# mrluin/TextualDegRemoval

Hardware: AMD Instinct MI355X
Metric: train images/sec (512x512, bs=4/GPU) (higher is better)
Workload: dtype f32 (3xbf16-split MFMA: 24-bit operand significands on the full fp32 exponent range, fp32 accumulate; unscaled gradients, no loss scale, no step-skip guard; tensors fp32 -- the MASA-encoder ResidualBlock activations / gradients as three bf16 planes whose sum IS the fp32 value, bit for bit)

## Files before the change

### textualdegremoval_amd/csrc/tdr_common.h

```cpp
#pragma once
#include <hip/hip_runtime.h>
#include <stdint.h>
#include <stdio.h>
#include <string.h>

#define TDR_OK 0
#define TDR_ERR_ARG (-1)
#define TDR_ERR_HIP (-2)
#define TDR_ERR_UNSUPPORTED (-3)

void tdr_set_error(const char* fmt, ...);

#define TDR_REQUIRE(cond, ...)                     \
    do {                                           \
        if (!(cond)) {                             \
            tdr_set_error(__VA_ARGS__);            \
            return TDR_ERR_ARG;                    \
        }                                          \
    } while (0)

#define TDR_LAUNCH_CHECK(name)                                                         \
    do {                                                                               \
        hipError_t e__ = hipGetLastError();                                            \
        if (e__ != hipSuccess) {                                                       \
            tdr_set_error("%s: launch failed: %s", name, hipGetErrorString(e__));      \
            return TDR_ERR_HIP;                                                        \
        }                                                                              \
    } while (0)

struct TdrConvDesc;
int tdr_conv_forward_bx3(const TdrConvDesc* d, void* stream);

static inline int tdr_cdiv(long a, long b) { return (int)((a + b - 1) / b); }

#include <stdlib.h>
#ifdef TDR_TUNING_KNOBS
static inline const char* tdr_tune_env(const char* name) { return getenv(name); }
#else
static inline const char* tdr_tune_env(const char*) { return nullptr; }
#endif

typedef __attribute__((ext_vector_type(16))) float f32x16;
typedef __attribute__((ext_vector_type(4))) float f32x4;

__device__ __forceinline__ float wave_sum(float v) {
#pragma unroll
    for (int o = 32; o > 0; o >>= 1) v += __shfl_xor(v, o, 64);
    return v;
}
template <int CTRL>
__device__ __forceinline__ float dpp_perm(float v) {
    return __builtin_bit_cast(float, __builtin_amdgcn_update_dpp(0, __builtin_bit_cast(int, v), CTRL, 0xf, 0xf, true));
}
__device__ __forceinline__ float wave_sum_dpp(float v) {
    v += dpp_perm<0xB1>(v);
    v += dpp_perm<0x4E>(v);
    v += dpp_perm<0x141>(v);
    v += dpp_perm<0x140>(v);
    const int b = __builtin_bit_cast(int, v);
    return (__builtin_bit_cast(float, __builtin_amdgcn_readlane(b, 0)) + __builtin_bit_cast(float, __builtin_amdgcn_readlane(b, 16))) +
           (__builtin_bit_cast(float, __builtin_amdgcn_readlane(b, 32)) + __builtin_bit_cast(float, __builtin_amdgcn_readlane(b, 48)));
}
__device__ __forceinline__ float wave_max(float v) {
#pragma unroll
    for (int o = 32; o > 0; o >>= 1) v = fmaxf(v, __shfl_xor(v, o, 64));
    return v;
}

typedef float tdr_f32x2 __attribute__((ext_vector_type(2)));
typedef _Float16 tdr_f16x2 __attribute__((ext_vector_type(2)));
template <bool PIN = true>
__device__ __forceinline__ void tdr_split2_f16(float x0, float x1, unsigned& h, unsigned& m) {
    if constexpr (PIN) asm volatile("" : "+v"(x0), "+v"(x1));
    const tdr_f32x2 xv = {x0, x1};
    h = __builtin_bit_cast(unsigned, __builtin_convertvector(xv, tdr_f16x2));
    const float neg1 = -1.0f;
    asm("v_fma_mixlo_f16 %0, %1, %2, %3 op_sel:[0,0,0] op_sel_hi:[1,0,0]" : "=v"(m) : "v"(h), "v"(neg1), "v"(x0));
    asm("v_fma_mixhi_f16 %0, %1, %2, %3 op_sel:[1,0,0] op_sel_hi:[1,0,0]" : "+v"(m) : "v"(h), "v"(neg1), "v"(x1));
}

typedef __bf16 tdr_bf16x2 __attribute__((ext_vector_type(2)));
template <bool PIN = true>
__device__ __forceinline__ void tdr_split3_bf16(float x0, float x1, unsigned& h, unsigned& m, unsigned& l) {
    if constexpr (PIN) asm volatile("" : "+v"(x0), "+v"(x1));
    const tdr_f32x2 xv = {x0, x1};
    h = __builtin_bit_cast(unsigned, __builtin_convertvector(xv, tdr_bf16x2));
    const float r0 = x0 - __builtin_bit_cast(float, h << 16), r1 = x1 - __builtin_bit_cast(float, h & 0xffff0000u);
    const tdr_f32x2 rv = {r0, r1};
    m = __builtin_bit_cast(unsigned, __builtin_convertvector(rv, tdr_bf16x2));
    const tdr_f32x2 sv = {r0 - __builtin_bit_cast(float, m << 16), r1 - __builtin_bit_cast(float, m & 0xffff0000u)};
    l = __builtin_bit_cast(unsigned, __builtin_convertvector(sv, tdr_bf16x2));
}
```

### textualdegremoval_amd/csrc/tdr_conv_mfma.hip

```cpp
#include "tdr_common.h"
#include "tdr_conv_epi.h"
#include "tdr_pack.h"
#include "../../include/tdr.h"

namespace {

constexpr int cmax(int a, int b) { return a > b ? a : b; }
constexpr int plane_elems(int NT, int TW, int KH, int S, int D) {
    return (((NT * 32 / TW) - 1) * S + (KH - 1) * D + 1) * ((TW - 1) * S + (KH - 1) * D + 1);
}
constexpr int max_plane(int NT, int KH, int S, int D) {
    return cmax(plane_elems(NT, 8, KH, S, D), cmax(plane_elems(NT, 16, KH, S, D), plane_elems(NT, 32, KH, S, D)));
}

template <int KH, int S, int D, int CK, int WM, int TM, int TN, int EPI, bool GATE>
__global__ __launch_bounds__(256) void conv_mfma_kernel(ConvArgs a) {
    constexpr int WN = 4 / WM;
    constexpr int BM = 32 * TM * WM;
    constexpr int NT = TN * WN;
    constexpr int TAPS = KH * KH;
    constexpr int KC = CK * TAPS;
    constexpr int MAXPIT = (max_plane(NT, KH, S, D) + 63) / 64;
    constexpr int CPW = CK / 4;
    constexpr int W4 = KC * BM / 4;
// ... 96 lines not shown
    const int abase = kk * BM + wm * TM * 32 + j;

    f32x16 acc[TM][TN];
#pragma unroll
    for (int tm = 0; tm < TM; ++tm)
#pragma unroll
        for (int tn = 0; tn < TN; ++tn)
#pragma unroll
            for (int r = 0; r < 16; ++r) acc[tm][tn][r] = 0.f;

    load_chunk(0);
    for (int ch = 0; ch < nchunks; ++ch) {
        {
            __syncthreads();
            store_chunk(ch);
            __syncthreads();
        }
        if (ch + 1 < nchunks) load_chunk(ch + 1);
#pragma unroll
        for (int tap = 0; tap < TAPS; ++tap) {
            const int tapoff = (tap / KH) * D * LW + (tap % KH) * D;
#pragma unroll
            for (int c2 = 0; c2 < CK / 2; ++c2) {
                float af[TM], bf[TN];
#pragma unroll
                for (int tm = 0; tm < TM; ++tm)
                    af[tm] = s_w[abase + (tap * CK + 2 * c2) * BM + tm * 32];
#pragma unroll
                for (int tn = 0; tn < TN; ++tn)
                    bf[tn] = s_in[bbase[tn] + 2 * c2 * plane + tapoff];
#pragma unroll
                for (int tm = 0; tm < TM; ++tm)
#pragma unroll
                    for (int tn = 0; tn < TN; ++tn)
                        acc[tm][tn] = __builtin_amdgcn_mfma_f32_32x32x2f32(af[tm], bf[tn], acc[tm][tn], 0, 0, 0);
            }
        }
    }

    conv_epilogue<TM, TN, EPI>(a, acc, n, m0, wm, wn, oy0, ox0, j, kk);
}

template <int KH, int S, int D, int CK, int WM, int TM, int TN, int EPI, bool GATE>
int launch_cfg(const ConvArgs& a, int N, hipStream_t st) {
    constexpr int WN = 4 / WM;
    constexpr int BM = 32 * TM * WM;
    constexpr int NT = TN * WN;
    constexpr int KC = CK * KH * KH;
    const int TW = 1 << a.tw_log2, SR = 32 >> a.tw_log2, TH = NT * SR;
    const int LH = (TH - 1) * S + (KH - 1) * D + 1, LW = (TW - 1) * S + (KH - 1) * D + 1;
    const size_t lds = (size_t)(KC * BM + CK * LH * LW) * sizeof(float);
    ConvArgs b = a;
    b.tiles_x = tdr_cdiv(a.OW, TW);
    const int tiles_y = tdr_cdiv(a.OH, TH);
    dim3 grid(b.tiles_x * tiles_y, tdr_cdiv(a.Cout, BM), N);
    auto kern = conv_mfma_kernel<KH, S, D, CK, WM, TM, TN, EPI, GATE>;
    static bool attr_set = false;
    if (!attr_set) {
        (void)hipFuncSetAttribute(reinterpret_cast<const void*>(kern), hipFuncAttributeMaxDynamicSharedMemorySize, 160 * 1024);
        attr_set = true;
    }
    hipLaunchKernelGGL(kern, grid, dim3(256), lds, st, b);
    TDR_LAUNCH_CHECK("conv_mfma_kernel");
    return TDR_OK;
}

template <int KH, int S, int D, int CK, int EPI, bool GATE>
int launch_shape(const ConvArgs& a, int N, hipStream_t st) {
    const long pix = (long)a.OH * a.OW;
    auto blocks = [&](int bm, int bn) { return (long)tdr_cdiv(a.Cout, bm) * tdr_cdiv(pix, bn) * N; };
    if (a.Cout <= 32) {
        if (blocks(32, 256) < 256) return launch_cfg<KH, S, D, CK, 1, 1, 1, EPI, GATE>(a, N, st);
        return launch_cfg<KH, S, D, CK, 1, 1, 2, EPI, GATE>(a, N, st);
    }
    if (a.Cout > 64 && blocks(128, 128) >= 512) return launch_cfg<KH, S, D, CK, 2, 2, 2, EPI, GATE>(a, N, st);
    if (blocks(64, 128) >= 512) return launch_cfg<KH, S, D, CK, 2, 1, 2, EPI, GATE>(a, N, st);
    return launch_cfg<KH, S, D, CK, 2, 1, 1, EPI, GATE>(a, N, st);
}

__global__ void pack_weights_kernel(const float* __restrict__ w, int Cout, int Cin, int KH, int mode, int CK,
                                    int M, int Kch, int KHe, int Mpad, long total, float* __restrict__ wp) {
    for (long i = blockIdx.x * (long)blockDim.x + threadIdx.x; i < total; i += (long)gridDim.x * blockDim.x)
        wp[i] = tdr_pack_f32_elem(w, Cin, KH, mode, CK, M, Kch, KHe, Mpad, i);
}

__global__ void pack_patches_kernel(const float* __restrict__ blk, int G, int C, int BH, int BW, int PH, int PW, int pstep,
                                    int dil, int off, int CK, int Mpad, long per_b, long total, float* __restrict__ wp) {
    for (long i = blockIdx.x * (long)blockDim.x + threadIdx.x; i < total; i += (long)gridDim.x * blockDim.x) {
        const long b = i / per_b;
        long r = i % per_b;
        const int m = (int)(r % Mpad); r /= Mpad;
        const int ck = (int)(r % CK); r /= CK;
        const int tap = (int)(r % 9);
        const int chunk = (int)(r / 9);
        const int c = chunk * CK + ck;
        float v = 0.f;
        if (m < G * PH * PW && c < C) {
            const int g = m / (PH * PW), q = m % (PH * PW);
            const int py = q / PW, px = q % PW;
            const int y = py * pstep + (tap / 3) * dil + off, x = px * pstep + (tap % 3) * dil + off;
            v = blk[(((b * G + g) * C + c) * BH + y) * BW + x];
        }
        wp[i] = v;
    }
}

}

extern "C" int tdr_conv_ck(int KH_eff) { return KH_eff == 1 ? 32 : (KH_eff == 2 ? 16 : 8); }

extern "C" int64_t tdr_packed_weight_floats(int M, int Kch, int KH_eff) {
    const int CK = tdr_conv_ck(KH_eff);
    const long Mpad = (M + 31) / 32 * 32;
    return (long)((Kch + CK - 1) / CK) * KH_eff * KH_eff * CK * Mpad;
}

extern "C" int tdr_pack_weights(const float* w, int Cout, int Cin, int KH, int mode, float* wp, void* stream) {
    TDR_REQUIRE(w && wp, "tdr_pack_weights: null pointer");
    TDR_REQUIRE(mode >= 0 && mode <= 3, "tdr_pack_weights: bad mode %d", mode);
    int M, Kch, KHe;
    if (mode == 0) { M = Cout; Kch = Cin; KHe = KH; }
    else if (mode == 1) { M = Cin; Kch = Cout; KHe = KH; }
    else if (mode == 2) { TDR_REQUIRE(KH == 2, "mode 2 needs a 2x2 kernel"); M = 4 * Cin; Kch = Cout; KHe = 1; }
    else { TDR_REQUIRE(KH == 3, "mode 3 needs a 3x3 kernel"); M = 4 * Cin; Kch = Cout; KHe = 2; }
    const int CK = tdr_conv_ck(KHe);
    const int Mpad = (M + 31) / 32 * 32;
    const long total = tdr_packed_weight_floats(M, Kch, KHe);
    const int blocks = (int)((total + 255) / 256 < 4096 ? (total + 255) / 256 : 4096);
    hipLaunchKernelGGL(pack_weights_kernel, dim3(blocks), dim3(256), 0, (hipStream_t)stream, w, Cout, Cin, KH, mode, CK,
                       M, Kch, KHe, Mpad, total, wp);
    TDR_LAUNCH_CHECK("pack_weights_kernel");
    return TDR_OK;
}

extern "C" int tdr_pack_patches(const float* blk, int B, int G, int C, int BH, int BW, int PH, int PW, int pstep, int dil,
                                int off, float* wp, void* stream) {
    TDR_REQUIRE(blk && wp, "tdr_pack_patches: null pointer");
    const int CK = 8;
    const int Mpad = (G * PH * PW + 31) / 32 * 32;
    const long per_b = (long)((C + CK - 1) / CK) * 9 * CK * Mpad;
    const long total = per_b * B;
    const int blocks = (int)((total + 255) / 256 < 8192 ? (total + 255) / 256 : 8192);
    hipLaunchKernelGGL(pack_patches_kernel, dim3(blocks), dim3(256), 0, (hipStream_t)stream, blk, G, C, BH, BW, PH, PW,
                       pstep, dil, off, CK, Mpad, per_b, total, wp);
    TDR_LAUNCH_CHECK("pack_patches_kernel");
    return TDR_OK;
}

extern "C" int tdr_conv_forward(const TdrConvDesc* d, void* stream) {
    TDR_REQUIRE(d && d->in && d->wp && d->out, "tdr_conv_forward: null pointer");
    TDR_REQUIRE(d->N > 0 && d->Cin > 0 && d->Cout > 0 && d->OH > 0 && d->OW > 0, "tdr_conv_forward: bad shape");
    TDR_REQUIRE(d->Mpad % 32 == 0 && d->Mpad >= d->Cout, "tdr_conv_forward: Mpad %d invalid for Cout %d", d->Mpad, d->Cout);
    TDR_REQUIRE(d->epi != EPI_GATEBWD || d->aux, "tdr_conv_forward: GATEBWD needs aux");
    if (d->wp_fmt >= 1 && d->wp_fmt <= 3) return tdr_conv_forward_bx3(d, stream);
    TDR_REQUIRE(d->wp_fmt == 0, "tdr_conv_forward: unknown wp_fmt %d", d->wp_fmt);
    ConvArgs a;
    a.in = d->in; a.in_ns = d->in_ns; a.Cin = d->Cin; a.H = d->H; a.W = d->W;
    a.wp = (const float*)d->wp; a.wp_ns = d->wp_ns; a.Mpad = d->Mpad; a.Cout = d->Cout;
    a.out = d->out; a.out_ns = d->out_ns; a.OH = d->OH; a.OW = d->OW;
    a.pad = d->pad;
    a.tw_log2 = d->OW >= 24 ? 5 : (d->OW >= 12 ? 4 : 3);
    a.tiles_x = 0;
    a.kscale = d->kscale; a.kscale_ns = d->kscale_ns;
    a.gate_off = (long)d->Cin * d->H * d->W;
    a.bias = d->bias; a.bias_ns = d->bias_ns; a.scale = d->scale; a.scale_ns = d->scale_ns;
    a.bias2 = d->bias2; a.bias2_ns = d->bias2_ns; a.bias2_mul = d->bias2_mul;
    a.res = d->res; a.res_ns = d->res_ns; a.mask = d->mask; a.mask_ns = d->mask_ns;
    a.aux = d->aux; a.aux_ns = d->aux_ns; a.relu = d->relu;
    a.vec_epi = 0; a.single_buf = 0; a.scheme = 0;
    hipStream_t st = (hipStream_t)stream;
    const int N = d->N;
    const int key = d->KH * 1000 + d->stride * 100 + d->dil * 10 + d->epi;
    const bool g = d->gate != 0;
    switch (key) {
        case 1110: return g ? launch_shape<1, 1, 1, 32, EPI_STD, true>(a, N, st)
                            : launch_shape<1, 1, 1, 32, EPI_STD, false>(a, N, st);
        case 1111: if (!g) return launch_shape<1, 1, 1, 32, EPI_GATEBWD, false>(a, N, st); break;
        case 1112: if (!g) return launch_shape<1, 1, 1, 32, EPI_PSHUF, false>(a, N, st); break;
        case 3110: if (!g) return launch_shape<3, 1, 1, 8, EPI_STD, false>(a, N, st); break;
        case 3112: if (!g) return launch_shape<3, 1, 1, 8, EPI_PSHUF, false>(a, N, st); break;
        case 3120: if (!g) return launch_shape<3, 1, 2, 8, EPI_STD, false>(a, N, st); break;
        case 3130: if (!g) return launch_shape<3, 1, 3, 8, EPI_STD, false>(a, N, st); break;
        case 3210: if (!g) return launch_shape<3, 2, 1, 8, EPI_STD, false>(a, N, st); break;
        case 2210: if (!g) return launch_shape<2, 2, 1, 16, EPI_STD, false>(a, N, st); break;
        case 2112: if (!g) return launch_shape<2, 1, 1, 16, EPI_PSHUF, false>(a, N, st); break;
        default: break;
    }
    tdr_set_error("tdr_conv_forward: unsupported (KH=%d stride=%d dil=%d epi=%d gate=%d)", d->KH, d->stride, d->dil,
                  d->epi, d->gate);
    return TDR_ERR_UNSUPPORTED;
}

namespace {
__global__ __launch_bounds__(256) void pack_multi_kernel(const TdrPackJob* __restrict__ jobs, int n_jobs) {
    int lo = 0, hi = n_jobs - 1;
    while (lo < hi) {
        const int mid = (lo + hi + 1) >> 1;
        if (jobs[mid].first_block <= (long)blockIdx.x) lo = mid; else hi = mid - 1;
    }
    const TdrPackJob jb = jobs[lo];
    const long i = ((long)blockIdx.x - jb.first_block) * 256 + threadIdx.x;
    if (i >= jb.total) return;
    if (jb.fmt == 0)
        reinterpret_cast<float*>(jb.wp)[i] = tdr_pack_f32_elem(jb.w, jb.Cin, jb.KH, jb.mode, jb.CK, jb.M, jb.Kch, jb.KHe, jb.Mx, i);
    else if (jb.fmt == 1 && jb.KHe == 3 && jb.mode == 0)
        tdr_pack_bx3_alltaps9<0>(jb.w, jb.Cin, jb.M, jb.Kch, jb.Mx, i, reinterpret_cast<uint4*>(jb.wp));
    else if (jb.fmt == 1 && jb.KHe == 3 && jb.mode == 1)
        tdr_pack_bx3_alltaps9<1>(jb.w, jb.Cin, jb.M, jb.Kch, jb.Mx, i, reinterpret_cast<uint4*>(jb.wp));
    else if (jb.fmt == 1)
        tdr_pack_bx3_frag(jb.w, jb.Cin, jb.KH, jb.mode, jb.M, jb.Kch, jb.KHe, jb.Mx, i, reinterpret_cast<uint4*>(jb.wp));
    else if (jb.mode == 0 && jb.KHe == 1)
        tdr_pack_hx2_fwd_alltaps<1>(jb.w, jb.Cin, jb.M, jb.Kch, jb.Mx, i, reinterpret_cast<uint4*>(jb.wp));
    else if (jb.mode == 0 && jb.KHe == 2)
        tdr_pack_hx2_fwd_alltaps<4>(jb.w, jb.Cin, jb.M, jb.Kch, jb.Mx, i, reinterpret_cast<uint4*>(jb.wp));
    else if (jb.mode == 0 && jb.KHe == 3)
        tdr_pack_hx2_fwd_alltaps<9>(jb.w, jb.Cin, jb.M, jb.Kch, jb.Mx, i, reinterpret_cast<uint4*>(jb.wp));
    else
        tdr_pack_hx2_frag(jb.w, jb.Cin, jb.KH, jb.mode, jb.M, jb.Kch, jb.KHe, jb.Mx, i, reinterpret_cast<uint4*>(jb.wp));
}
}

extern "C" int tdr_pack_job_init(TdrPackJob* job, const float* w, int Cout, int Cin, int KH, int mode, int fmt, void* wp) {
    TDR_REQUIRE(job && w && wp, "tdr_pack_job_init: null pointer");
    TDR_REQUIRE(mode >= 0 && mode <= 3 && fmt >= 0 && fmt <= 2, "tdr_pack_job_init: bad mode/fmt");
    int M, Kch, KHe;
    if (mode == 0) { M = Cout; Kch = Cin; KHe = KH; }
    else if (mode == 1) { M = Cin; Kch = Cout; KHe = KH; }
    else if (mode == 2) { TDR_REQUIRE(KH == 2, "mode 2 needs a 2x2 kernel"); M = 4 * Cin; Kch = Cout; KHe = 1; }
    else { TDR_REQUIRE(KH == 3, "mode 3 needs a 3x3 kernel"); M = 4 * Cin; Kch = Cout; KHe = 2; }
    job->w = w; job->wp = wp; job->Cout = Cout; job->Cin = Cin; job->KH = KH; job->mode = mode; job->fmt = fmt;
    job->M = M; job->Kch = Kch; job->KHe = KHe;
    if (fmt == 0) {
        job->CK = tdr_conv_ck(KHe);
        job->Mx = (M + 31) / 32 * 32;
        job->total = tdr_packed_weight_floats(M, Kch, KHe);
    } else {
        job->CK = 16;
        job->Mx = (M + 31) / 32;
        job->total = (long)((Kch + 15) / 16) * KHe * KHe * job->Mx * 64;
        if (fmt == 2 && mode == 0 && KHe >= 1 && KHe <= 3) job->total = (long)((Kch + 15) / 16) * job->Mx * 64;
        if (fmt == 1 && KHe == 3 && mode <= 1) job->total = (long)((Kch + 15) / 16) * job->Mx * 64;
    }
    job->first_block = 0;
    return TDR_OK;
}

extern "C" int tdr_pack_weights_multi(const TdrPackJob* jobs_dev, int n_jobs, int64_t total_blocks, void* stream) {
    TDR_REQUIRE(jobs_dev && n_jobs > 0 && total_blocks > 0 && total_blocks < (1LL << 31), "tdr_pack_weights_multi: bad argument");
    hipLaunchKernelGGL(pack_multi_kernel, dim3((unsigned)total_blocks), dim3(256), 0, (hipStream_t)stream, jobs_dev, n_jobs);
    TDR_LAUNCH_CHECK("pack_multi_kernel");
    return TDR_OK;
}
```

### textualdegremoval_amd/csrc/tdr_wgrad_common.h

```cpp
#pragma once
#include "tdr_common.h"

struct TdrWgradDesc;

struct WgArgs {
    const float* in; long in_ns; int Cin, H, W; long gate_off;
    const float* dout; long dout_ns; int Cout, OH, OW;
    int pad, tw_log2, tiles_x, tiles_y, tpi , tps , spi ;
    float* part;
    float* dbpart;
    int scheme;
    const void* grp_tab;
    int grp_bpp;
    int grp_pairs;
};

struct WgPlan { int tw_log2, tiles_x, tiles_y, tpi, tps, spi, cfg, WKw, BMc, BNc; };

bool tdr_wgrad_bx3_supported(const TdrWgradDesc* d);
WgPlan tdr_wgrad_bx3_plan(const TdrWgradDesc* d);
int tdr_wgrad_bx3_launch(const WgArgs& a, const WgPlan& p, const TdrWgradDesc* d, hipStream_t st);

bool tdr_wgrad_s2_supported(const TdrWgradDesc* d);
WgPlan tdr_wgrad_s2_plan(const TdrWgradDesc* d);
int tdr_wgrad_s2_launch(const WgArgs& a, const WgPlan& p, const TdrWgradDesc* d, hipStream_t st);

bool tdr_wgrad_1x1_supported(const TdrWgradDesc* d);
WgPlan tdr_wgrad_1x1_plan(const TdrWgradDesc* d);
int tdr_wgrad_1x1_launch(const WgArgs& a, const WgPlan& p, const TdrWgradDesc* d, hipStream_t st);
```

### textualdegremoval_amd/csrc/tdr_wgrad_mfma.hip

```cpp
#include <stdio.h>
#include <stdlib.h>
#include "tdr_common.h"
#include "tdr_wgrad_common.h"
#include "../../include/tdr.h"

namespace {

constexpr int wg_plane(int TW, int KH, int S) { return (((64 / TW) - 1) * S + KH) * ((TW - 1) * S + KH); }
constexpr int wg_cmax(int a, int b) { return a > b ? a : b; }
constexpr int wg_max_plane(int KH, int S) {
    return wg_cmax(wg_plane(8, KH, S), wg_cmax(wg_plane(16, KH, S), wg_plane(32, KH, S)));
}

template <int KH, int S, int WMw, int WNw, int WKw, int TMW, int TNW, bool GATE>
__global__ __launch_bounds__(256) void wgrad_mfma_kernel(WgArgs a) {
    static_assert(WMw * WNw * WKw == 4, "4 waves");
    constexpr int TAPS = KH * KH;
    constexpr int BMc = 32 * TMW * WMw, BNc = 32 * TNW * WNw;
    constexpr int MAXPIT = (wg_max_plane(KH, S) + 63) / 64;
    constexpr int DPT = BMc / 4;
    constexpr int IPT = BNc / 4;
    constexpr int KPW = 32 / WKw;

    extern __shared__ __attribute__((aligned(16))) float smem[];
// ... 30 lines not shown
    for (int i = 0; i < DPT; ++i) rdsum[i] = 0.f;
    float ri[IPT][MAXPIT];
    float ri2[GATE ? IPT : 1][GATE ? MAXPIT : 1];
    bool dok_r = false;
    unsigned iok_r = 0;
    auto load_tile = [&](int t) {
        const int ty = t / a.tiles_x, tx = t % a.tiles_x;
        const int oy0 = ty * (64 >> a.tw_log2), ox0 = tx * TW;
        const int oy = oy0 + dpy, ox = ox0 + dpx;
        dok_r = oy < a.OH && ox < a.OW;
        const long doff = dok_r ? (long)oy * a.OW + ox : 0;
#pragma unroll
        for (int i = 0; i < DPT; ++i) {
            const int co = min(co0 + wave + 4 * i, a.Cout - 1);
            rd[i] = do_n[(long)co * HWo + doff];
        }
        const int iy0 = oy0 * S - a.pad, ix0 = ox0 * S - a.pad;
        iok_r = 0;
#pragma unroll
        for (int it = 0; it < MAXPIT; ++it) {
            const int gy = iy0 + pr[it], gx = ix0 + pc[it];
            const bool ok = pr[it] >= 0 && gy >= 0 && gy < a.H && gx >= 0 && gx < a.W;
            iok_r |= (ok ? 1u : 0u) << it;
            const long off = ok ? (long)gy * a.W + gx : 0;
#pragma unroll
            for (int i = 0; i < IPT; ++i) {
                const int ci = min(ci0 + wave + 4 * i, a.Cin - 1);
                ri[i][it] = in_n[(long)ci * HWin + off];
                if (GATE) ri2[i][it] = in_n[(long)ci * HWin + off + a.gate_off];
            }
        }
    };
    auto store_tile = [&]() {
#pragma unroll
        for (int i = 0; i < DPT; ++i) {
            const float dv = (dok_r && co0 + wave + 4 * i < a.Cout) ? rd[i] : 0.f;
            s_d[(wave + 4 * i) * 65 + lane] = dv;
            rdsum[i] += dv;
        }
#pragma unroll
        for (int it = 0; it < MAXPIT; ++it)
            if (pr[it] >= 0) {
#pragma unroll
                for (int i = 0; i < IPT; ++i) {
                    float v = ri[i][it];
                    if (GATE) v *= ri2[i][it];
                    s_i[(wave + 4 * i) * planeP + lane + 64 * it] =
                        (((iok_r >> it) & 1u) && ci0 + wave + 4 * i < a.Cin) ? v : 0.f;
                }
            }
    };

    f32x16 acc[TMW][TNW][TAPS];
#pragma unroll
    for (int x = 0; x < TMW; ++x)
#pragma unroll
        for (int y = 0; y < TNW; ++y)
#pragma unroll
            for (int t = 0; t < TAPS; ++t)
#pragma unroll
                for (int r = 0; r < 16; ++r) acc[x][y][t][r] = 0.f;

    const int abase = (wm * TMW * 32 + j) * 65 + kk;
    const int bbase = (wn * TNW * 32 + j) * planeP + kk * S;

    if (t_begin < t_end) load_tile(t_begin);
    for (int t = t_begin; t < t_end; ++t) {
        __syncthreads();
        store_tile();
        __syncthreads();
        if (t + 1 < t_end) load_tile(t + 1);
#pragma unroll
        for (int q = 0; q < KPW; ++q) {
            const int k2 = wk * KPW + q;
            const int p0 = 2 * k2;
            const int py0 = p0 >> a.tw_log2, px0 = p0 & (TW - 1);
            const int pixoff = py0 * S * LW + px0 * S;
            float af[TMW];
#pragma unroll
            for (int x = 0; x < TMW; ++x) af[x] = s_d[abase + x * 32 * 65 + p0];
#pragma unroll
            for (int tap = 0; tap < TAPS; ++tap) {
                const int toff = pixoff + (tap / KH) * LW + (tap % KH);
#pragma unroll
                for (int y = 0; y < TNW; ++y) {
                    const float bf = s_i[bbase + y * 32 * planeP + toff];
#pragma unroll
                    for (int x = 0; x < TMW; ++x)
                        acc[x][y][tap] = __builtin_amdgcn_mfma_f32_32x32x2f32(af[x], bf, acc[x][y][tap], 0, 0, 0);
                }
            }
        }
    }

    if (a.dbpart && blockIdx.z == 0) {
#pragma unroll
        for (int i = 0; i < DPT; ++i) {
            const float sv = wave_sum(rdsum[i]);
            const int co = co0 + wave + 4 * i;
            if (lane == 0 && co < a.Cout) a.dbpart[(long)split * a.Cout + co] = sv;
        }
    }
    float* part = a.part + ((long)split * WKw + wk) * a.Cout * a.Cin * TAPS;
#pragma unroll
    for (int x = 0; x < TMW; ++x)
#pragma unroll
        for (int y = 0; y < TNW; ++y) {
            const int ci = ci0 + (wn * TNW + y) * 32 + j;
            if (ci >= a.Cin) continue;
#pragma unroll
            for (int r = 0; r < 16; ++r) {
                const int co = co0 + (wm * TMW + x) * 32 + (r & 3) + 8 * (r >> 2) + 4 * kk;
                if (co >= a.Cout) continue;
#pragma unroll
                for (int tap = 0; tap < TAPS; ++tap) part[((long)co * a.Cin + ci) * TAPS + tap] = acc[x][y][tap][r];
            }
        }
}

template <int KL>
__global__ __launch_bounds__(64 * KL) void wgrad_reduce_kernel(const float* __restrict__ part, long elems, int per_group,
                                                               float* __restrict__ out, int nb_main,
                                                               const float* __restrict__ part2, long elems2, int per_group2,
                                                               float* __restrict__ out2) {
    __shared__ float red[KL][64];
    const int lane = threadIdx.x & 63, kl = threadIdx.x >> 6;
    const bool second = (int)blockIdx.x >= nb_main;
    if (second && blockIdx.y != 0) return;
    const float* pbase = second ? part2 : part;
    const long ne = second ? elems2 : elems;
    const int pg = second ? per_group2 : per_group;
    float* o = second ? out2 : out;
    const long e = ((int)blockIdx.x - (second ? nb_main : 0)) * 64L + lane;
    const long ec = e < ne ? e : ne - 1;
    const float* p = pbase + (second ? 0L : (long)blockIdx.y * pg * ne) + ec;
    float s0 = 0.f;
    for (int k = kl; k < pg; k += 8 * KL) {
        float v[8];
#pragma unroll
        for (int u = 0; u < 8; ++u) v[u] = k + u * KL < pg ? p[(long)(k + u * KL) * ne] : 0.f;
        s0 += ((v[0] + v[1]) + (v[2] + v[3])) + ((v[4] + v[5]) + (v[6] + v[7]));
    }
    red[kl][lane] = s0;
    __syncthreads();
    if (kl == 0 && e < ne) {
        float t = 0.f;
#pragma unroll
        for (int q = 0; q < KL; ++q) t += red[q][lane];
        o[(second ? 0L : (long)blockIdx.y * ne) + e] = t;
    }
}

WgPlan make_plan(const TdrWgradDesc* d) {
    if (tdr_wgrad_1x1_supported(d)) return tdr_wgrad_1x1_plan(d);
    if (d->math >= 1 && tdr_wgrad_bx3_supported(d)) return tdr_wgrad_bx3_plan(d);
    if (tdr_wgrad_s2_supported(d)) return tdr_wgrad_s2_plan(d);
    WgPlan p;
    p.tw_log2 = d->OW >= 24 ? 5 : (d->OW >= 12 ? 4 : 3);
    const int TW = 1 << p.tw_log2, TH = 64 >> p.tw_log2;
    p.tiles_x = tdr_cdiv(d->OW, TW);
    p.tiles_y = tdr_cdiv(d->OH, TH);
    p.tpi = p.tiles_x * p.tiles_y;
    if (d->KH == 1) {
        if (d->Cout >= 128 && d->Cin >= 128) p.cfg = 0;
        else if (d->Cin <= 32) p.cfg = d->Cout <= 32 ? 3 : 1;
        else p.cfg = 2;
    } else if (d->KH == 3 && d->stride == 1) {
        p.cfg = (d->Cin <= 32 && d->Cout <= 32) ? 3 : 2;
    } else {
        p.cfg = 2;
    }
    static const int bm[4] = {128, 64, 64, 32}, bn[4] = {128, 32, 64, 32}, wk[4] = {1, 4, 1, 4};
    p.BMc = bm[p.cfg]; p.BNc = bn[p.cfg]; p.WKw = wk[p.cfg];
    const long out_tiles = (long)tdr_cdiv(d->Cout, p.BMc) * tdr_cdiv(d->Cin, p.BNc);
    long want = (p.WKw > 1 ? 256 : 512) / out_tiles;
    if (want < 1) want = 1;
    long spi = (want + d->N - 1) / d->N;
    if (spi > p.tpi / 4) spi = p.tpi / 4;
    if (spi < 1) spi = 1;
    p.tps = tdr_cdiv(p.tpi, spi);
    p.spi = tdr_cdiv(p.tpi, p.tps);
    return p;
}

template <int KH, int S, int WMw, int WNw, int WKw, int TMW, int TNW, bool GATE>
int launch_wg(const WgArgs& a, const WgPlan& p, int N, hipStream_t st) {
    constexpr int BMc = 32 * TMW * WMw, BNc = 32 * TNW * WNw;
    const int TW = 1 << a.tw_log2;
    const int LH = ((64 >> a.tw_log2) - 1) * S + KH, LW = (TW - 1) * S + KH;
    const size_t lds = (size_t)(BMc * 65 + BNc * ((LH * LW) | 1)) * sizeof(float);
    dim3 grid(N * p.spi, tdr_cdiv(a.Cout, BMc), tdr_cdiv(a.Cin, BNc));
    auto kern = wgrad_mfma_kernel<KH, S, WMw, WNw, WKw, TMW, TNW, GATE>;
    static bool attr_set = false;
    if (!attr_set) {
        (void)hipFuncSetAttribute(reinterpret_cast<const void*>(kern), hipFuncAttributeMaxDynamicSharedMemorySize, 160 * 1024);
        attr_set = true;
    }
    hipLaunchKernelGGL(kern, grid, dim3(256), lds, st, a);
    TDR_LAUNCH_CHECK("wgrad_mfma_kernel");
    return TDR_OK;
}

}

extern "C" int64_t tdr_wgrad_ws_floats(const TdrWgradDesc* d) {
    const WgPlan p = make_plan(d);
    return (int64_t)d->N * p.spi * p.WKw * d->Cout * d->Cin * d->KH * d->KH + (int64_t)d->N * p.spi * d->Cout;
}

extern "C" int tdr_conv_wgrad(const TdrWgradDesc* d, void* stream) {
    TDR_REQUIRE(d && d->in && d->dout && d->g && d->ws, "tdr_conv_wgrad: null pointer");
    const WgPlan p = make_plan(d);
    const int64_t need = tdr_wgrad_ws_floats(d);
    TDR_REQUIRE(d->ws_floats >= need, "tdr_conv_wgrad: workspace too small (%lld < %lld)", (long long)d->ws_floats,
                (long long)need);
    WgArgs a;
    a.in = d->in; a.in_ns = d->in_ns; a.Cin = d->Cin; a.H = d->H; a.W = d->W;
    a.gate_off = (long)d->Cin * d->H * d->W;
    a.dout = d->dout; a.dout_ns = d->dout_ns; a.Cout = d->Cout; a.OH = d->OH; a.OW = d->OW;
    a.grp_tab = nullptr; a.grp_bpp = 0; a.grp_pairs = 0;
    a.pad = d->pad; a.tw_log2 = p.tw_log2; a.tiles_x = p.tiles_x; a.tiles_y = p.tiles_y; a.tpi = p.tpi; a.tps = p.tps; a.spi = p.spi;
    const bool direct = !d->db && (d->per_image ? p.spi : d->N * p.spi) * p.WKw == 1;
    a.part = direct ? d->g : d->ws;
    a.dbpart = d->db ? d->ws + (int64_t)d->N * p.spi * p.WKw * d->Cout * d->Cin * d->KH * d->KH : nullptr;
    hipStream_t st = (hipStream_t)stream;
    const bool g = d->gate != 0;
    int rc = TDR_ERR_UNSUPPORTED;
    const int key = d->KH * 10 + d->stride;
    a.scheme = d->math == 3 ? 2 : (d->math == 2 ? 1 : 0);
    static const bool dbg = tdr_tune_env("TDR_WG_DEBUG") != nullptr;
    if (dbg && !(d->math >= 1 && tdr_wgrad_bx3_supported(d)) && !tdr_wgrad_s2_supported(d))
        fprintf(stderr, "[tdr] exact wgrad: math %d N %d %d->%d @%dx%d k%d s%d pad %d gate %d per_image %d in_ns %ld dout_ns %ld\n", d->math,
                d->N, d->Cin, d->Cout, d->H, d->W, d->KH, d->stride, d->pad, d->gate, d->per_image, (long)d->in_ns, (long)d->dout_ns);
    if (tdr_wgrad_1x1_supported(d)) {
        rc = tdr_wgrad_1x1_launch(a, p, d, st);
    } else if (d->math >= 1 && tdr_wgrad_bx3_supported(d)) {
        rc = tdr_wgrad_bx3_launch(a, p, d, st);
    } else if (tdr_wgrad_s2_supported(d)) {
        rc = tdr_wgrad_s2_launch(a, p, d, st);
    } else if (key == 11) {
        switch (p.cfg) {
            case 0: rc = g ? launch_wg<1, 1, 2, 2, 1, 2, 2, true>(a, p, d->N, st) : launch_wg<1, 1, 2, 2, 1, 2, 2, false>(a, p, d->N, st); break;
            case 1: rc = g ? launch_wg<1, 1, 1, 1, 4, 2, 1, true>(a, p, d->N, st) : launch_wg<1, 1, 1, 1, 4, 2, 1, false>(a, p, d->N, st); break;
            case 2: rc = g ? launch_wg<1, 1, 2, 2, 1, 1, 1, true>(a, p, d->N, st) : launch_wg<1, 1, 2, 2, 1, 1, 1, false>(a, p, d->N, st); break;
            default: rc = g ? launch_wg<1, 1, 1, 1, 4, 1, 1, true>(a, p, d->N, st) : launch_wg<1, 1, 1, 1, 4, 1, 1, false>(a, p, d->N, st); break;
        }
    } else if (key == 31 && !g) {
        rc = p.cfg == 3 ? launch_wg<3, 1, 1, 1, 4, 1, 1, false>(a, p, d->N, st) : launch_wg<3, 1, 2, 2, 1, 1, 1, false>(a, p, d->N, st);
    } else if (key == 32 && !g) {
        rc = launch_wg<3, 2, 2, 2, 1, 1, 1, false>(a, p, d->N, st);
    } else if (key == 22 && !g) {
        rc = launch_wg<2, 2, 2, 2, 1, 1, 1, false>(a, p, d->N, st);
    } else {
        tdr_set_error("tdr_conv_wgrad: unsupported (KH=%d stride=%d gate=%d)", d->KH, d->stride, d->gate);
        return TDR_ERR_UNSUPPORTED;
    }
    if (rc != TDR_OK || direct) return rc;
    const long elems = (long)d->Cout * d->Cin * d->KH * d->KH;
    const int groups = d->per_image ? d->N : 1;
    const int per_group = (d->per_image ? p.spi : d->N * p.spi) * p.WKw;
    const int nb_main = tdr_cdiv(elems, 64);
    const int nb2 = d->db ? tdr_cdiv(d->Cout, 64) : 0;
    const int pg2 = d->N * p.spi;
    const dim3 rgrid(nb_main + nb2, groups);
    if (per_group <= 8 && pg2 <= 8)
        hipLaunchKernelGGL(wgrad_reduce_kernel<1>, rgrid, dim3(64), 0, st, d->ws, elems, per_group, d->g, nb_main, a.dbpart,
                           (long)d->Cout, pg2, d->db);
    else if (per_group <= 64 && pg2 <= 64)
        hipLaunchKernelGGL(wgrad_reduce_kernel<4>, rgrid, dim3(256), 0, st, d->ws, elems, per_group, d->g, nb_main, a.dbpart,
                           (long)d->Cout, pg2, d->db);
    else
        hipLaunchKernelGGL(wgrad_reduce_kernel<16>, rgrid, dim3(1024), 0, st, d->ws, elems, per_group, d->g, nb_main, a.dbpart,
                           (long)d->Cout, pg2, d->db);
    TDR_LAUNCH_CHECK("wgrad_reduce_kernel");
    return TDR_OK;
}
```

Measured before the change: 60.54.

## Add direct-FMA kernels for thin-channel 3x3 conv forward and weight gradient

Adds dedicated scalar-FMA kernels for 3x3 stride-1 convolutions where one side has at most 4 channels (e.g. image input/output layers), bypassing the padded MFMA path. Forward thin-in and thin-out kernels stage input rows in LDS and keep a register sliding window. A thin wgrad kernel reduces per-wave partials with DPP. This removes the waste of padding tiny channel counts up to MFMA tile sizes, at the cost of new code paths with their own precision and alignment handling.

```diff
diff --git a/textualdegremoval_amd/csrc/tdr_common.h b/textualdegremoval_amd/csrc/tdr_common.h
--- a/textualdegremoval_amd/csrc/tdr_common.h
+++ b/textualdegremoval_amd/csrc/tdr_common.h
@@ -30,6 +30,8 @@
 
 struct TdrConvDesc;
 int tdr_conv_forward_bx3(const TdrConvDesc* d, void* stream);
+bool tdr_conv_thin_supported(const TdrConvDesc* d);
+int tdr_conv_thin_forward(const TdrConvDesc* d, void* stream);
 
 static inline int tdr_cdiv(long a, long b) { return (int)((a + b - 1) / b); }
 
diff --git a/textualdegremoval_amd/csrc/tdr_conv_mfma.hip b/textualdegremoval_amd/csrc/tdr_conv_mfma.hip
--- a/textualdegremoval_amd/csrc/tdr_conv_mfma.hip
+++ b/textualdegremoval_amd/csrc/tdr_conv_mfma.hip
@@ -272,6 +272,7 @@
     TDR_REQUIRE(d->N > 0 && d->Cin > 0 && d->Cout > 0 && d->OH > 0 && d->OW > 0, "tdr_conv_forward: bad shape");
     TDR_REQUIRE(d->Mpad % 32 == 0 && d->Mpad >= d->Cout, "tdr_conv_forward: Mpad %d invalid for Cout %d", d->Mpad, d->Cout);
     TDR_REQUIRE(d->epi != EPI_GATEBWD || d->aux, "tdr_conv_forward: GATEBWD needs aux");
+    if (tdr_conv_thin_supported(d)) return tdr_conv_thin_forward(d, stream);
     if (d->wp_fmt >= 1 && d->wp_fmt <= 3) return tdr_conv_forward_bx3(d, stream);
     TDR_REQUIRE(d->wp_fmt == 0, "tdr_conv_forward: unknown wp_fmt %d", d->wp_fmt);
     ConvArgs a;
diff --git a/textualdegremoval_amd/csrc/tdr_conv_thin.hip b/textualdegremoval_amd/csrc/tdr_conv_thin.hip
--- /dev/null
+++ b/textualdegremoval_amd/csrc/tdr_conv_thin.hip
@@ -0,0 +1,428 @@
+#include "tdr_common.h"
+#include "tdr_wgrad_common.h"
+#include "../../include/tdr.h"
+
+namespace {
+
+constexpr int TW = 128, TH = 8;
+constexpr int LP = TW + 4;
+
+struct ThinArgs {
+    const float* in; long in_ns; int Cin, H, W;
+    const void* wp; int wp_fmt, Mpad, Cout;
+    float* out; long out_ns;
+    const float* bias; long bias_ns;
+    const float* res; long res_ns;
+    int relu, vec, tiles_x;
+};
+
+__device__ __forceinline__ float bf16_bits_to_f32(unsigned short b) { return __builtin_bit_cast(float, (unsigned)b << 16); }
+
+__device__ __forceinline__ float thin_weight(const void* wp, int fmt, int Mpad, int m, int c, int tap) {
+    if (fmt == 0) return reinterpret_cast<const float*>(wp)[(((long)(c >> 3) * 9 + tap) * 8 + (c & 7)) * Mpad + m];
+    const int MT = Mpad >> 5;
+    const long frag = (((long)(c >> 4) * 9 + tap) * MT + (m >> 5)) * 3 * 64 + (m & 31) + 32 * ((c >> 3) & 1);
+    const unsigned short* f = reinterpret_cast<const unsigned short*>(wp) + frag * 8 + (c & 7);
+    return (bf16_bits_to_f32(f[0]) + bf16_bits_to_f32(f[64 * 8])) + bf16_bits_to_f32(f[128 * 8]);
+}
+
+template <int ROWS, int COLS, int PITCH, int WAVES>
+__device__ __forceinline__ void stage_rows(float* s, const float* __restrict__ src, long HW, int nch, int H, int W, int y0, int x0,
+                                           int wave, int lane) {
+    constexpr int NJ = (COLS + 63) / 64;
+    int gx[NJ];
+    bool okx[NJ];
+#pragma unroll
+    for (int q = 0; q < NJ; ++q) {
+        const int j = lane + 64 * q, x = x0 - 1 + j;
+        okx[q] = j < COLS && x >= 0 && x < W;
+        gx[q] = okx[q] ? x : 0;
+    }
+    for (int row = wave; row < nch * ROWS; row += WAVES) {
+        const int c = row / ROWS, r = row - c * ROWS;
+        const int y = y0 - 1 + r;
+        const bool oky = y >= 0 && y < H;
+        const float* p = src + (long)c * HW + (long)(oky ? y : 0) * W;
+        float v[NJ];
+#pragma unroll
+        for (int q = 0; q < NJ; ++q) v[q] = p[gx[q]];
+#pragma unroll
+        for (int q = 0; q < NJ; ++q)
+            if (lane + 64 * q < COLS) s[row * PITCH + lane + 64 * q] = (oky && okx[q]) ? v[q] : 0.f;
+    }
+}
+
+__device__ __forceinline__ void thin_store(const ThinArgs& a, int n, int m, int y, int x, float (&v)[4]) {
+    const long off = (long)m * a.H * a.W + (long)y * a.W + x;
+    float* o = a.out + (long)n * a.out_ns + off;
+    const float* r = a.res ? a.res + (long)n * a.res_ns + off : nullptr;
+    if (a.bias) {
+        const float b = a.bias[(long)n * a.bias_ns + m];
+#pragma unroll
+        for (int p = 0; p < 4; ++p) v[p] += b;
+    }
+    if (a.vec) {
+        if (r) {
+            const f32x4 rv = *reinterpret_cast<const f32x4*>(r);
+#pragma unroll
+            for (int p = 0; p < 4; ++p) v[p] += rv[p];
+        }
+        if (a.relu) {
+#pragma unroll
+            for (int p = 0; p < 4; ++p) v[p] = fmaxf(v[p], 0.f);
+        }
+        const f32x4 ov = {v[0], v[1], v[2], v[3]};
+        *reinterpret_cast<f32x4*>(o) = ov;
+    } else {
+#pragma unroll
+        for (int p = 0; p < 4; ++p)
+            if (x + p < a.W) {
+                float t = v[p];
+                if (r) t += r[p];
+                if (a.relu) t = fmaxf(t, 0.f);
+                o[p] = t;
+            }
+    }
+}
+
+template <int CIN>
+__global__ __launch_bounds__(256, 2) void thin_in_kernel(ThinArgs a) {
+    extern __shared__ __attribute__((aligned(16))) float smem[];
+    float* s_in = smem;
+    float* s_w = smem + CIN * (TH + 2) * LP;
+    const int tid = threadIdx.x, lane = tid & 63, wave = __builtin_amdgcn_readfirstlane(tid >> 6);
+    const int tx = blockIdx.x % a.tiles_x, ty = blockIdx.x / a.tiles_x, n = blockIdx.z;
+    const int x0 = tx * TW, y0 = ty * TH;
+    for (int i = tid; i < a.Cout * CIN * 9; i += 256) {
+        const int co = i & 15;
+        int r = i >> 4;
+        const int c = r % CIN; r /= CIN;
+        const int tap = r % 9, cg = r / 9;
+        s_w[i] = thin_weight(a.wp, a.wp_fmt, a.Mpad, cg * 16 + co, c, tap);
+    }
+    stage_rows<TH + 2, TW + 2, LP, 4>(s_in, a.in + (long)n * a.in_ns, (long)a.H * a.W, CIN, a.H, a.W, y0, x0, wave, lane);
+    __syncthreads();
+    const int lx = tid & 31, ly = tid >> 5;
+    const int x = x0 + 4 * lx, y = y0 + ly;
+    if (y >= a.H || x >= a.W) return;
+    float xin[CIN][3][6];
+#pragma unroll
+    for (int c = 0; c < CIN; ++c)
+#pragma unroll
+        for (int r = 0; r < 3; ++r) {
+            const float* p = s_in + (c * (TH + 2) + ly + r) * LP + 4 * lx;
+            const f32x4 q = *reinterpret_cast<const f32x4*>(p);
+            const tdr_f32x2 q2 = *reinterpret_cast<const tdr_f32x2*>(p + 4);
+            xin[c][r][0] = q[0]; xin[c][r][1] = q[1]; xin[c][r][2] = q[2]; xin[c][r][3] = q[3];
+            xin[c][r][4] = q2[0]; xin[c][r][5] = q2[1];
+        }
+#pragma unroll 1
+    for (int g4 = 0; g4 < (a.Cout >> 2); ++g4) {
+        float acc[4][4];
+#pragma unroll
+        for (int co = 0; co < 4; ++co)
+#pragma unroll
+            for (int p = 0; p < 4; ++p) acc[co][p] = 0.f;
+#pragma unroll
+        for (int tap = 0; tap < 9; ++tap)
+#pragma unroll
+            for (int c = 0; c < CIN; ++c) {
+                const f32x4 wv = *reinterpret_cast<const f32x4*>(s_w + (((g4 >> 2) * 9 + tap) * CIN + c) * 16 + (g4 & 3) * 4);
+#pragma unroll
+                for (int co = 0; co < 4; ++co)
+#pragma unroll
+                    for (int p = 0; p < 4; ++p) acc[co][p] = __builtin_fmaf(wv[co], xin[c][tap / 3][tap % 3 + p], acc[co][p]);
+            }
+#pragma unroll
+        for (int co = 0; co < 4; ++co) thin_store(a, n, g4 * 4 + co, y, x, acc[co]);
+    }
+}
+
+template <int COUT>
+__global__ __launch_bounds__(256) void thin_out_kernel(ThinArgs a) {
+    extern __shared__ __attribute__((aligned(16))) float smem[];
+    float* s_in = smem;
+    float* s_w = smem + 8 * (TH + 2) * LP;
+    const int tid = threadIdx.x, lane = tid & 63, wave = __builtin_amdgcn_readfirstlane(tid >> 6);
+    const int tx = blockIdx.x % a.tiles_x, ty = blockIdx.x / a.tiles_x, n = blockIdx.z;
+    const int x0 = tx * TW, y0 = ty * TH;
+    const long HW = (long)a.H * a.W;
+    for (int i = tid; i < a.Cin * 9 * 4; i += 256) {
+        const int co = i & 3, c8 = (i >> 2) & 7;
+        const int r = i >> 5;
+        const int tap = r % 9, ch = r / 9;
+        s_w[i] = co < COUT ? thin_weight(a.wp, a.wp_fmt, a.Mpad, co, ch * 8 + c8, tap) : 0.f;
+    }
+    const int lx = tid & 31, ly = tid >> 5;
+    const int x = x0 + 4 * lx, y = y0 + ly;
+    float acc[COUT][4];
+#pragma unroll
+    for (int co = 0; co < COUT; ++co)
+#pragma unroll
+        for (int p = 0; p < 4; ++p) acc[co][p] = 0.f;
+    const float* in_n = a.in + (long)n * a.in_ns;
+    for (int ch = 0; ch < (a.Cin >> 3); ++ch) {
+        __syncthreads();
+        stage_rows<TH + 2, TW + 2, LP, 4>(s_in, in_n + (long)ch * 8 * HW, HW, 8, a.H, a.W, y0, x0, wave, lane);
+        __syncthreads();
+#pragma unroll
+        for (int ky = 0; ky < 3; ++ky) {
+            float xr[8][6];
+#pragma unroll
+            for (int c = 0; c < 8; ++c) {
+                const float* p = s_in + (c * (TH + 2) + ly + ky) * LP + 4 * lx;
+                const f32x4 q = *reinterpret_cast<const f32x4*>(p);
+                const tdr_f32x2 q2 = *reinterpret_cast<const tdr_f32x2*>(p + 4);
+                xr[c][0] = q[0]; xr[c][1] = q[1]; xr[c][2] = q[2]; xr[c][3] = q[3]; xr[c][4] = q2[0]; xr[c][5] = q2[1];
+            }
+#pragma unroll
+            for (int kx = 0; kx < 3; ++kx)
+#pragma unroll
+                for (int c = 0; c < 8; ++c) {
+                    const f32x4 wv = *reinterpret_cast<const f32x4*>(s_w + ((ch * 9 + ky * 3 + kx) * 8 + c) * 4);
+#pragma unroll
+                    for (int co = 0; co < COUT; ++co)
+#pragma unroll
+                        for (int p = 0; p < 4; ++p) acc[co][p] = __builtin_fmaf(wv[co], xr[c][kx + p], acc[co][p]);
+                }
+        }
+    }
+    if (y >= a.H || x >= a.W) return;
+#pragma unroll
+    for (int co = 0; co < COUT; ++co) thin_store(a, n, co, y, x, acc[co]);
+}
+
+constexpr int WGW = 256, WGR = 8, WGP = WGW + 8;
+
+struct ThinWgArgs {
+    const float* thin; long thin_ns; int TC;
+    const float* wide; long wide_ns; int WC;
+    int H, W, flip, vec, strips_x, spi, rows;
+    float* part; float* dbpart;
+};
+
+template <int TC>
+__global__ __launch_bounds__(512) void thin_wgrad_kernel(ThinWgArgs a) {
+    __shared__ __attribute__((aligned(16))) float s_t[TC * (WGR + 2) * WGP];
+    const int tid = threadIdx.x, lane = tid & 63, wave = __builtin_amdgcn_readfirstlane(tid >> 6);
+    const int split = blockIdx.x, n = split / a.spi, s = split % a.spi;
+    const int sx = s % a.strips_x, sy = s / a.strips_x;
+    const int x0 = sx * WGW, r_begin = sy * a.rows, r_end = min(r_begin + a.rows, a.H);
+    const int wc0 = blockIdx.y * 32 + wave * 4;
+    const bool active = wc0 < a.WC;
+    const long HW = (long)a.H * a.W;
+    const int x = x0 + 4 * lane;
+    const bool xok = x < a.W;
+    const float* tn = a.thin + (long)n * a.thin_ns;
+    const float* wn = a.wide + (long)n * a.wide_ns + (long)min(wc0, a.WC - 4) * HW;
+
+    auto load_wide = [&](int y, f32x4 (&v)[4]) {
+#pragma unroll
+        for (int c = 0; c < 4; ++c) {
+            const float* p = wn + (long)c * HW + (long)y * a.W;
+            if (a.vec) {
+                const f32x4 t = *reinterpret_cast<const f32x4*>(p + (xok ? x : 0));
+                const f32x4 z = {0.f, 0.f, 0.f, 0.f};
+                v[c] = xok ? t : z;
+            } else {
+#pragma unroll
+                for (int q = 0; q < 4; ++q) {
+                    const bool ok = x + q < a.W;
+                    const float t = p[ok ? x + q : 0];
+                    v[c][q] = ok ? t : 0.f;
+                }
+            }
+        }
+    };
+
+    float acc[4][TC][9];
+    float dbw[4], dbt[TC];
+#pragma unroll
+    for (int c = 0; c < 4; ++c) {
+        dbw[c] = 0.f;
+#pragma unroll
+        for (int t = 0; t < TC; ++t)
+#pragma unroll
+            for (int k = 0; k < 9; ++k) acc[c][t][k] = 0.f;
+    }
+#pragma unroll
+    for (int t = 0; t < TC; ++t) dbt[t] = 0.f;
+
+    f32x4 wv[4], wnext[4];
+    if (active && r_begin < r_end) load_wide(r_begin, wnext);
+    for (int rc = r_begin; rc < r_end; rc += WGR) {
+        __syncthreads();
+        stage_rows<WGR + 2, WGW + 2, WGP, 8>(s_t, tn, HW, TC, a.H, a.W, rc, x0, wave, lane);
+        __syncthreads();
+        if (!active) continue;
+        const int nr = min(WGR, r_end - rc);
+        for (int ry = 0; ry < nr; ++ry) {
+#pragma unroll
+            for (int c = 0; c < 4; ++c) wv[c] = wnext[c];
+            if (rc + ry + 1 < r_end) load_wide(rc + ry + 1, wnext);
+#pragma unroll
+            for (int c = 0; c < 4; ++c)
+#pragma unroll
+                for (int p = 0; p < 4; ++p) dbw[c] += wv[c][p];
+#pragma unroll
+            for (int r = 0; r < 3; ++r) {
+                float tv[TC][6];
+#pragma unroll
+                for (int t = 0; t < TC; ++t) {
+                    const float* p = s_t + (t * (WGR + 2) + ry + r) * WGP + 4 * lane;
+                    const f32x4 q = *reinterpret_cast<const f32x4*>(p);
+                    const tdr_f32x2 q2 = *reinterpret_cast<const tdr_f32x2*>(p + 4);
+                    tv[t][0] = q[0]; tv[t][1] = q[1]; tv[t][2] = q[2]; tv[t][3] = q[3]; tv[t][4] = q2[0]; tv[t][5] = q2[1];
+                }
+#pragma unroll
+                for (int c = 0; c < 4; ++c)
+#pragma unroll
+                    for (int t = 0; t < TC; ++t)
+#pragma unroll
+                        for (int kx = 0; kx < 3; ++kx)
+#pragma unroll
+                            for (int p = 0; p < 4; ++p)
+                                acc[c][t][r * 3 + kx] = __builtin_fmaf(wv[c][p], tv[t][kx + p], acc[c][t][r * 3 + kx]);
+                if (r == 1) {
+#pragma unroll
+                    for (int t = 0; t < TC; ++t)
+#pragma unroll
+                        for (int p = 0; p < 4; ++p) dbt[t] += tv[t][1 + p];
+                }
+            }
+        }
+    }
+    if (!active) return;
+    constexpr int NE = 4 * TC * 9, NR = (NE + 63) / 64;
+    float outv[NR];
+#pragma unroll
+    for (int r = 0; r < NR; ++r) outv[r] = 0.f;
+#pragma unroll
+    for (int c = 0; c < 4; ++c)
+#pragma unroll
+        for (int t = 0; t < TC; ++t)
+#pragma unroll
+            for (int k = 0; k < 9; ++k) {
+                const int e = (c * TC + t) * 9 + k;
+                const float sv = wave_sum_dpp(acc[c][t][k]);
+                if (lane == (e & 63)) outv[e >> 6] = sv;
+            }
+    const int Cout = a.flip ? a.TC : a.WC, Cin = a.flip ? a.WC : a.TC;
+    float* part = a.part + (long)split * Cout * Cin * 9;
+#pragma unroll
+    for (int r = 0; r < NR; ++r) {
+        const int e = r * 64 + lane;
+        if (e < NE) {
+            const int k = e % 9, t = (e / 9) % TC, c = e / (9 * TC);
+            const long dst = a.flip ? ((long)t * Cin + wc0 + c) * 9 + (8 - k) : ((long)(wc0 + c) * Cin + t) * 9 + k;
+            part[dst] = outv[r];
+        }
+    }
+    if (a.dbpart) {
+        if (!a.flip) {
+#pragma unroll
+            for (int c = 0; c < 4; ++c) {
+                const float sv = wave_sum_dpp(dbw[c]);
+                if (lane == 0) a.dbpart[(long)split * Cout + wc0 + c] = sv;
+            }
+        } else if (wc0 == 0) {
+#pragma unroll
+            for (int t = 0; t < TC; ++t) {
+                const float sv = wave_sum_dpp(dbt[t]);
+                if (lane == 0) a.dbpart[(long)split * Cout + t] = sv;
+            }
+        }
+    }
+}
+
+inline bool al16(const void* p) { return (reinterpret_cast<uintptr_t>(p) & 15) == 0; }
+
+template <typename K>
+int thin_launch(K kern, const char* name, const ThinArgs& a, int N, size_t lds, hipStream_t st) {
+    ThinArgs b = a;
+    b.tiles_x = tdr_cdiv(a.W, TW);
+    dim3 grid(b.tiles_x * tdr_cdiv(a.H, TH), 1, N);
+    hipLaunchKernelGGL(kern, grid, dim3(256), lds, st, b);
+    TDR_LAUNCH_CHECK(name);
+    return TDR_OK;
+}
+
+}
+
+bool tdr_conv_thin_supported(const TdrConvDesc* d) {
+    if (d->KH != 3 || d->stride != 1 || d->dil != 1 || d->pad != 1 || d->OH != d->H || d->OW != d->W) return false;
+    if (d->epi != 0 || d->gate || d->kscale || d->scale || d->bias2 || d->mask || d->aux || d->wp_ns != 0) return false;
+    if (d->relu != 0 && d->relu != 1) return false;
+    if (d->wp_fmt != 0 && d->wp_fmt != 1) return false;
+    const bool thin_in = d->Cin <= 4 && d->Cout % 16 == 0;
+    const bool thin_out = d->Cout <= 4 && d->Cin % 16 == 0;
+    return (thin_in || thin_out) && d->Cin <= 128 && d->Cout <= 128;
+}
+
+int tdr_conv_thin_forward(const TdrConvDesc* d, void* stream) {
+    ThinArgs a;
+    a.in = d->in; a.in_ns = d->in_ns; a.Cin = d->Cin; a.H = d->H; a.W = d->W;
+    a.wp = d->wp; a.wp_fmt = d->wp_fmt; a.Mpad = d->Mpad; a.Cout = d->Cout;
+    a.out = d->out; a.out_ns = d->out_ns;
+    a.bias = d->bias; a.bias_ns = d->bias_ns; a.res = d->res; a.res_ns = d->res_ns;
+    a.relu = d->relu; a.tiles_x = 0;
+    a.vec = (d->W % 4 == 0 && d->out_ns % 4 == 0 && al16(d->out) && (!d->res || (d->res_ns % 4 == 0 && al16(d->res)))) ? 1 : 0;
+    hipStream_t st = (hipStream_t)stream;
+    if (d->Cin <= 4) {
+        const size_t lds = (size_t)(d->Cin * (TH + 2) * LP + d->Cout * d->Cin * 9) * sizeof(float);
+        switch (d->Cin) {
+            case 1: return thin_launch(thin_in_kernel<1>, "thin_in_kernel", a, d->N, lds, st);
+            case 2: return thin_launch(thin_in_kernel<2>, "thin_in_kernel", a, d->N, lds, st);
+            case 3: return thin_launch(thin_in_kernel<3>, "thin_in_kernel", a, d->N, lds, st);
+            default: return thin_launch(thin_in_kernel<4>, "thin_in_kernel", a, d->N, lds, st);
+        }
+    }
+    const size_t lds = (size_t)(8 * (TH + 2) * LP + d->Cin * 9 * 4) * sizeof(float);
+    switch (d->Cout) {
+        case 1: return thin_launch(thin_out_kernel<1>, "thin_out_kernel", a, d->N, lds, st);
+        case 2: return thin_launch(thin_out_kernel<2>, "thin_out_kernel", a, d->N, lds, st);
+        case 3: return thin_launch(thin_out_kernel<3>, "thin_out_kernel", a, d->N, lds, st);
+        default: return thin_launch(thin_out_kernel<4>, "thin_out_kernel", a, d->N, lds, st);
+    }
+}
+
+bool tdr_wgrad_thin_supported(const TdrWgradDesc* d) {
+    if (d->KH != 3 || d->stride != 1 || d->pad != 1 || d->gate || d->per_image || d->OH != d->H || d->OW != d->W) return false;
+    if (d->math != 0 && d->math != 1) return false;
+    return (d->Cin <= 4 && d->Cout % 16 == 0) || (d->Cout <= 4 && d->Cin % 16 == 0);
+}
+
+WgPlan tdr_wgrad_thin_plan(const TdrWgradDesc* d) {
+    WgPlan p;
+    p.tw_log2 = 0; p.cfg = 0; p.BMc = d->Cout; p.BNc = d->Cin; p.WKw = 1;
+    const int wide = d->Cin <= 4 ? d->Cout : d->Cin;
+    p.tiles_x = tdr_cdiv(d->W, WGW);
+    long rs = 256 / ((long)d->N * p.tiles_x * tdr_cdiv(wide, 32));
+    if (rs < 1) rs = 1;
+    p.tps = (tdr_cdiv(d->H, rs) + WGR - 1) / WGR * WGR;
+    p.tiles_y = tdr_cdiv(d->H, p.tps);
+    p.tpi = p.tiles_x * p.tiles_y;
+    p.spi = p.tpi;
+    return p;
+}
+
+int tdr_wgrad_thin_launch(const WgArgs& w, const WgPlan& p, const TdrWgradDesc* d, hipStream_t st) {
+    ThinWgArgs a;
+    const bool flip = d->Cin > 4;
+    a.flip = flip ? 1 : 0;
+    a.thin = flip ? d->dout : d->in; a.thin_ns = flip ? d->dout_ns : d->in_ns; a.TC = flip ? d->Cout : d->Cin;
+    a.wide = flip ? d->in : d->dout; a.wide_ns = flip ? d->in_ns : d->dout_ns; a.WC = flip ? d->Cin : d->Cout;
+    a.H = d->H; a.W = d->W;
+    a.vec = (d->W % 4 == 0 && a.wide_ns % 4 == 0 && al16(a.wide)) ? 1 : 0;
+    a.strips_x = p.tiles_x; a.spi = p.spi; a.rows = p.tps;
+    a.part = w.part; a.dbpart = w.dbpart;
+    dim3 grid(d->N * p.spi, tdr_cdiv(a.WC, 32));
+    switch (a.TC) {
+        case 1: hipLaunchKernelGGL(thin_wgrad_kernel<1>, grid, dim3(512), 0, st, a); break;
+        case 2: hipLaunchKernelGGL(thin_wgrad_kernel<2>, grid, dim3(512), 0, st, a); break;
+        case 3: hipLaunchKernelGGL(thin_wgrad_kernel<3>, grid, dim3(512), 0, st, a); break;
+        default: hipLaunchKernelGGL(thin_wgrad_kernel<4>, grid, dim3(512), 0, st, a); break;
+    }
+    TDR_LAUNCH_CHECK("thin_wgrad_kernel");
+    return TDR_OK;
+}
diff --git a/textualdegremoval_amd/csrc/tdr_wgrad_common.h b/textualdegremoval_amd/csrc/tdr_wgrad_common.h
--- a/textualdegremoval_amd/csrc/tdr_wgrad_common.h
+++ b/textualdegremoval_amd/csrc/tdr_wgrad_common.h
@@ -28,3 +28,7 @@
 bool tdr_wgrad_1x1_supported(const TdrWgradDesc* d);
 WgPlan tdr_wgrad_1x1_plan(const TdrWgradDesc* d);
 int tdr_wgrad_1x1_launch(const WgArgs& a, const WgPlan& p, const TdrWgradDesc* d, hipStream_t st);
+
+bool tdr_wgrad_thin_supported(const TdrWgradDesc* d);
+WgPlan tdr_wgrad_thin_plan(const TdrWgradDesc* d);
+int tdr_wgrad_thin_launch(const WgArgs& a, const WgPlan& p, const TdrWgradDesc* d, hipStream_t st);
diff --git a/textualdegremoval_amd/csrc/tdr_wgrad_mfma.hip b/textualdegremoval_amd/csrc/tdr_wgrad_mfma.hip
--- a/textualdegremoval_amd/csrc/tdr_wgrad_mfma.hip
+++ b/textualdegremoval_amd/csrc/tdr_wgrad_mfma.hip
@@ -206,6 +206,7 @@
 }
 
 WgPlan make_plan(const TdrWgradDesc* d) {
+    if (tdr_wgrad_thin_supported(d)) return tdr_wgrad_thin_plan(d);
     if (tdr_wgrad_1x1_supported(d)) return tdr_wgrad_1x1_plan(d);
     if (d->math >= 1 && tdr_wgrad_bx3_supported(d)) return tdr_wgrad_bx3_plan(d);
     if (tdr_wgrad_s2_supported(d)) return tdr_wgrad_s2_plan(d);
@@ -283,10 +284,12 @@
     const int key = d->KH * 10 + d->stride;
     a.scheme = d->math == 3 ? 2 : (d->math == 2 ? 1 : 0);
     static const bool dbg = tdr_tune_env("TDR_WG_DEBUG") != nullptr;
-    if (dbg && !(d->math >= 1 && tdr_wgrad_bx3_supported(d)) && !tdr_wgrad_s2_supported(d))
+    if (dbg && !tdr_wgrad_thin_supported(d) && !(d->math >= 1 && tdr_wgrad_bx3_supported(d)) && !tdr_wgrad_s2_supported(d))
         fprintf(stderr, "[tdr] exact wgrad: math %d N %d %d->%d @%dx%d k%d s%d pad %d gate %d per_image %d in_ns %ld dout_ns %ld\n", d->math,
                 d->N, d->Cin, d->Cout, d->H, d->W, d->KH, d->stride, d->pad, d->gate, d->per_image, (long)d->in_ns, (long)d->dout_ns);
-    if (tdr_wgrad_1x1_supported(d)) {
+    if (tdr_wgrad_thin_supported(d)) {
+        rc = tdr_wgrad_thin_launch(a, p, d, st);
+    } else if (tdr_wgrad_1x1_supported(d)) {
         rc = tdr_wgrad_1x1_launch(a, p, d, st);
     } else if (d->math >= 1 && tdr_wgrad_bx3_supported(d)) {
         rc = tdr_wgrad_bx3_launch(a, p, d, st);
```

Result: no change. 61.01 (median of 6 runs) (+0.8%).
